# bioinformatics-ua/polus

Measured on AMD Instinct MI355X. Metric: train samples/sec BioBERT-base NER seq256, higher is better.
Workload: dtype bf16; 1 GPU; BERT-base (L=12,H=768,A=12,I=3072,V=28996) token classification C=4, seq_len=256, 64 samples/GPU, AdamW lr 5e-5 wd 0.01 warm-up 10%, dropout 0.1 (hidden + attention) (BASELINE.json configs[2] per-GPU shape), random-init weights; global_batch=64, seq_len=256, parallelism=dp1, grad_allreduce=none

## Files before the change

polus_amd/csrc/attention.hip:

```cpp
#include "common.h"

namespace {

constexpr int D = 64;
constexpr int BLK = 64;
constexpr float MASK_NEG = -10000.0f;
constexpr float LOG2E = 1.4426950408889634f, LN2 = 0.6931471805599453f;

template <typename T> struct TileCfg;
template <> struct TileCfg<bf16_t> { static constexpr int RS = 160, EPC = 8, LOG_CPR = 3, NLOAD = 2; };
template <> struct TileCfg<float> { static constexpr int RS = 288, EPC = 4, LOG_CPR = 4, NLOAD = 4; };

template <typename T, int NT = 256>
__device__ __forceinline__ void tile_load(unsigned char* tile, const T* __restrict__ base, long ld, int row0,
                                          int nrows, int col0, int tid) {
    constexpr int LOG = TileCfg<T>::LOG_CPR;
#pragma unroll
    for (int k = 0; k < TileCfg<T>::NLOAD; ++k) {
        int c = tid + NT * k;
        int r = c >> LOG, ch = c & ((1 << LOG) - 1);
        uint4 v = make_uint4(0, 0, 0, 0);
        if (row0 + r < nrows)
            v = *reinterpret_cast<const uint4*>(base + (long)(row0 + r) * ld + col0 + ch * TileCfg<T>::EPC);
        *reinterpret_cast<uint4*>(tile + r * TileCfg<T>::RS + ch * 16) = v;
    }
}

template <typename T>
__device__ __forceinline__ void frag_global(Frag<T>& f, const T* __restrict__ p, bool valid);
template <>
__device__ __forceinline__ void frag_global<bf16_t>(Frag<bf16_t>& f, const bf16_t* __restrict__ p, bool valid) {
    uint4 v = make_uint4(0, 0, 0, 0);
    if (valid) v = *reinterpret_cast<const uint4*>(p);
    f.v = __builtin_bit_cast(bf16x8, v);
}
template <>
__device__ __forceinline__ void frag_global<float>(Frag<float>& f, const float* __restrict__ p, bool valid) {
    float4 a = make_float4(0, 0, 0, 0), b = a;
    if (valid) { a = *reinterpret_cast<const float4*>(p); b = *reinterpret_cast<const float4*>(p + 4); }
    f.v[0] = a.x; f.v[1] = a.y; f.v[2] = a.z; f.v[3] = a.w;
    f.v[4] = b.x; f.v[5] = b.y; f.v[6] = b.z; f.v[7] = b.w;
}

template <typename T>
__device__ __forceinline__ void frag_row(Frag<T>& f, const unsigned char* tile, int row, int sub, int g) {
    frag_load_row(f, tile + row * TileCfg<T>::RS + (sub * 32 + 8 * g) * (int)sizeof(T));
}

__device__ __forceinline__ void frag_tr(Frag<bf16_t>& f, const unsigned char* tile, int kb, int d0, int i, int g) {
    const unsigned char* p = tile + (kb + 4 * g + (i >> 2)) * 160 + (d0 + 4 * (i & 3)) * 2;
    s16x4 lo = lds_tr16(p);
    s16x4 hi = lds_tr16(p + 16 * 160);
    typedef short s16x8 __attribute__((ext_vector_type(8)));
    s16x8 w = {lo[0], lo[1], lo[2], lo[3], hi[0], hi[1], hi[2], hi[3]};
    f.v = __builtin_bit_cast(bf16x8, w);
}
__device__ __forceinline__ void frag_tr(Frag<float>& f, const unsigned char* tile, int kb, int d0, int i, int g) {
#pragma unroll
    for (int j = 0; j < 8; ++j)
        f.v[j] = *reinterpret_cast<const float*>(tile + (kb + 16 * (j >> 2) + 4 * g + (j & 3)) * 288 + (d0 + i) * 4);
}

__device__ __forceinline__ void frag_from_acc(Frag<bf16_t>& f, const f32x4& t0, const f32x4& t1) {
    f.v[0] = (bf16_t)t0[0]; f.v[1] = (bf16_t)t0[1]; f.v[2] = (bf16_t)t0[2]; f.v[3] = (bf16_t)t0[3];
    f.v[4] = (bf16_t)t1[0]; f.v[5] = (bf16_t)t1[1]; f.v[6] = (bf16_t)t1[2]; f.v[7] = (bf16_t)t1[3];
}
__device__ __forceinline__ void frag_from_acc(Frag<float>& f, const f32x4& t0, const f32x4& t1) {
    f.v[0] = t0[0]; f.v[1] = t0[1]; f.v[2] = t0[2]; f.v[3] = t0[3];
    f.v[4] = t1[0]; f.v[5] = t1[1]; f.v[6] = t1[2]; f.v[7] = t1[3];
}

__device__ __forceinline__ float col_max(float v) { v = fmaxf(v, __shfl_xor(v, 16, 64)); return fmaxf(v, __shfl_xor(v, 32, 64)); }
__device__ __forceinline__ float col_sum(float v) { v += __shfl_xor(v, 16, 64); return v + __shfl_xor(v, 32, 64); }

template <typename T>
__device__ __forceinline__ void store_acc_T(T* __restrict__ out, long ld, int row, int col0, const f32x4 (&o)[4],
                                            float mul, int g, bool valid) {
    if (!valid) return;
#pragma unroll
    for (int dt = 0; dt < 4; ++dt) {
        float v[4] = {o[dt][0] * mul, o[dt][1] * mul, o[dt][2] * mul, o[dt][3] * mul};
        store4<T>(out + (long)row * ld + col0 + dt * 16 + 4 * g, v);
    }
}

struct AttnArgs {
    const void* qkv; const int32_t* mask; void* ctx; float* lse;
    const void* dctx; const float* delta; void* dqkv;
    int B, S, A, H;
    float scale;
    unsigned drop_thresh, drop_seed;
    float drop_inv;
    const PolusDyn* dyn;
    int debug;
};

__device__ __forceinline__ float key_bias(const int32_t* mask, int b, int S, int key) {
    if (key >= S) return -INFINITY;
    if (!mask) return 0.0f;
    return (1.0f - (float)mask[(long)b * S + key]) * MASK_NEG;
}

template <typename T, int NW>
__global__ __launch_bounds__(64 * NW) void attn_fwd_kernel(AttnArgs p) {
    if (p.drop_thresh) p.drop_seed = polus_eff_seed(p.drop_seed, p.dyn);
    constexpr int QB = 16 * NW, NT = 64 * NW;
    extern __shared__ __attribute__((aligned(16))) unsigned char smem[];
    unsigned char* Kc = smem;
    unsigned char* Vc = smem + QB * TileCfg<T>::RS;
    float* kbc = reinterpret_cast<float*>(smem + 2 * QB * TileCfg<T>::RS);
    const int tid = threadIdx.x, lane = tid & 63, wid = tid >> 6, i = lane & 15, g = lane >> 4;
    const int q0 = blockIdx.x * QB, h = blockIdx.y, b = blockIdx.z;
    const int S = p.S, H = p.H;
    const long ld = 3L * H;
    const T* qkv = static_cast<const T*>(p.qkv) + (long)b * S * ld;
    const int q = q0 + wid * 16 + i;
    const bool qvalid = q < S;

    Frag<T> qf[2];
#pragma unroll
    for (int sub = 0; sub < 2; ++sub)
        frag_global<T>(qf[sub], qkv + (long)q * ld + h * D + sub * 32 + 8 * g, qvalid);

    const float scale2 = p.scale * LOG2E;
    float m = -1e30f, l = 0.f;
    f32x4 o[4];
#pragma unroll
    for (int dt = 0; dt < 4; ++dt) o[dt] = (f32x4){0.f, 0.f, 0.f, 0.f};

    for (int kc0 = 0; kc0 < S; kc0 += QB) {
        __syncthreads();
        tile_load<T, NT>(Kc, qkv, ld, kc0, S, H + h * D, tid);
        tile_load<T, NT>(Vc, qkv, ld, kc0, S, 2 * H + h * D, tid);
        if (tid < QB) kbc[tid] = key_bias(p.mask, b, S, kc0 + tid) * LOG2E;
        __syncthreads();
      for (int kb0 = kc0; kb0 < kc0 + QB && kb0 < S; kb0 += BLK) {
        const unsigned char* Kt = Kc + (kb0 - kc0) * TileCfg<T>::RS;
        const unsigned char* Vt = Vc + (kb0 - kc0) * TileCfg<T>::RS;
        const float* kbias = kbc + (kb0 - kc0);

        f32x4 s[4];
#pragma unroll
        for (int kt = 0; kt < 4; ++kt) {
            s[kt] = (f32x4){0.f, 0.f, 0.f, 0.f};
#pragma unroll
            for (int sub = 0; sub < 2; ++sub) {
                Frag<T> a;
                frag_row<T>(a, Kt, kt * 16 + i, sub, g);
                mma16(s[kt], a, qf[sub]);
            }
        }
        float mx = -INFINITY;
#pragma unroll
        for (int kt = 0; kt < 4; ++kt)
#pragma unroll
            for (int r = 0; r < 4; ++r) {
                s[kt][r] = fmaf(s[kt][r], scale2, kbias[kt * 16 + 4 * g + r]);
                mx = fmaxf(mx, s[kt][r]);
            }
        mx = col_max(mx);
        const float m_new = fmaxf(m, mx);
        const float alpha = __builtin_amdgcn_exp2f(m - m_new);
        float rs = 0.f;
#pragma unroll
        for (int kt = 0; kt < 4; ++kt)
#pragma unroll
            for (int r = 0; r < 4; ++r) { s[kt][r] = __builtin_amdgcn_exp2f(s[kt][r] - m_new); rs += s[kt][r]; }
        rs = col_sum(rs);
        l = l * alpha + rs;
        m = m_new;
#pragma unroll
        for (int dt = 0; dt < 4; ++dt)
#pragma unroll
            for (int r = 0; r < 4; ++r) o[dt][r] *= alpha;
        if (p.drop_thresh) {
            const unsigned rowb = (((unsigned)b * p.A + h) * S + (unsigned)q) * S + kb0 + 4 * g;
#pragma unroll
            for (int kt = 0; kt < 4; ++kt) {
                float t4[4] = {s[kt][0], s[kt][1], s[kt][2], s[kt][3]};
                polus_dropout_run<4>(t4, p.drop_seed, rowb + kt * 16, p.drop_thresh, p.drop_inv, (S & 3) == 0);
                s[kt] = (f32x4){t4[0], t4[1], t4[2], t4[3]};
            }
        }
// ... 19 lines not shown
typedef const __attribute__((address_space(1))) void* gptr_t;
__device__ __forceinline__ void dma16(const void* g, unsigned char* lds) {
    __builtin_amdgcn_global_load_lds((gptr_t)g, (lds_void_t*)lds, 16, 0, 0);
}
__device__ __forceinline__ void dma4(const void* g, unsigned char* lds) {
    __builtin_amdgcn_global_load_lds((gptr_t)g, (lds_void_t*)lds, 4, 0, 0);
}
template <int N> __device__ __forceinline__ void wait_vm() { asm volatile("s_waitcnt vmcnt(%0)" :: "n"(N) : "memory"); }
__device__ __forceinline__ void wait_lgkm() { asm volatile("s_waitcnt lgkmcnt(0)" ::: "memory"); }
template <int PPW> __device__ __forceinline__ void wait_blocks_left(int left) {
    if (left >= 3) wait_vm<3 * PPW>(); else if (left == 2) wait_vm<2 * PPW>(); else if (left == 1) wait_vm<PPW>(); else wait_vm<0>();
}
__device__ __forceinline__ float xor16(float v) {
    return __builtin_bit_cast(float, __builtin_amdgcn_ds_swizzle(__builtin_bit_cast(int, v), 0x401F));
}
__device__ __forceinline__ float col_max2(float v) {
    v = fmaxf(v, xor16(v));
    return fmaxf(v, __shfl_xor(v, 32, 64));
}
__device__ __forceinline__ float col_sum2(float v) {
    v += xor16(v);
    return v + __shfl_xor(v, 32, 64);
}

constexpr int FWD_RING = 4, FWD_STAGE = 2 * BLK * 128;
constexpr int FWD_MAX_S = 1024;

template <int NW>
__global__ __launch_bounds__(64 * NW, NW == 8 ? 4 : 2) void attn_fwd_dma_kernel(AttnArgs p) {
    typedef bf16_t T;
    constexpr int QB = 16 * NW, NT = 64 * NW, PPW = 16 / NW;
    if (p.drop_thresh) p.drop_seed = polus_eff_seed(p.drop_seed, p.dyn);
    extern __shared__ __attribute__((aligned(16))) unsigned char smem[];
    unsigned char* ring = smem;
    float* kbc = reinterpret_cast<float*>(smem + FWD_RING * FWD_STAGE);
    const int tid = threadIdx.x, lane = tid & 63, i = lane & 15, g = lane >> 4;
    const int wid = __builtin_amdgcn_readfirstlane(tid >> 6);
    const int q0 = blockIdx.x * QB, h = blockIdx.y, b = blockIdx.z;
    const int S = p.S, H = p.H;
    const long ld = 3L * H;
    const T* qkv = static_cast<const T*>(p.qkv) + (long)b * S * ld;
    const int q = q0 + wid * 16 + i;
    const int r8 = lane >> 3, src_chunk = ((lane & 7) ^ r8) * 8;

    auto issue_block = [&](int j) {
        unsigned char* st = ring + (j & 3) * FWD_STAGE;
#pragma unroll
        for (int e = 0; e < PPW; ++e) {
            const int piece = wid + e * NW;
            const int row = min(j * BLK + (piece & 7) * 8 + r8, S - 1);
            dma16(qkv + (long)row * ld + (piece < 8 ? H : 2 * H) + h * D + src_chunk, st + piece * 1024);
        }
    };
    const int nblk = (S + BLK - 1) / BLK;
    if (p.mask)
        for (int k0 = wid * 64; k0 < S; k0 += 64 * NW)
            dma4(p.mask + (long)b * S + min(k0 + lane, S - 1), reinterpret_cast<unsigned char*>(kbc) + k0 * 4);
    {
        unsigned char* qs = ring + 3 * FWD_STAGE;
#pragma unroll
        for (int e = 0; e < 2; ++e) {
            const int piece = wid + e * NW;
            dma16(qkv + (long)min(q0 + piece * 8 + r8, S - 1) * ld + h * D + src_chunk, qs + piece * 1024);
        }
    }
#pragma unroll
    for (int j = 0; j < 3; ++j) if (j < nblk) issue_block(j);
    wait_blocks_left<PPW>(min(nblk, 3));
    __builtin_amdgcn_s_barrier();
    Frag<T> qf[2];
    {
        const int row = wid * 16 + i;
#pragma unroll
        for (int sub = 0; sub < 2; ++sub)
            qf[sub].v = *reinterpret_cast<const bf16x8*>(ring + 3 * FWD_STAGE + row * 128 + (((sub * 4 + g) ^ (row & 7)) * 16));
    }
    for (int t = tid; t < nblk * BLK; t += NT) {
        float bias = 0.0f;
        if (p.mask) bias = (1.0f - (float)reinterpret_cast<const int*>(kbc)[t]) * MASK_NEG;
        kbc[t] = t < S ? bias * LOG2E : -INFINITY;
    }
    wait_lgkm();
    __builtin_amdgcn_s_barrier();
    if (nblk > 3) issue_block(3);
    int issued = min(nblk, 4);

    const float scale2 = p.scale * LOG2E;
    float m = -1e30f, l = 0.f;
    f32x4 o[4];
#pragma unroll
    for (int dt = 0; dt < 4; ++dt) o[dt] = (f32x4){0.f, 0.f, 0.f, 0.f};
    const int kx = i & 7;
    const int k_off0 = i * 128 + ((g ^ kx) * 16), k_off1 = i * 128 + (((4 + g) ^ kx) * 16);
    const int vrow = 4 * g + (i >> 2), vx = vrow & 7;
    const int v_base = vrow * 128 + (i & 1) * 8, v_c = (i & 3) >> 1;

    for (int j0 = 0; j0 < nblk; j0 += 2) {
        const bool two = j0 + 1 < nblk;
        f32x4 s[2][4];
#pragma unroll
        for (int jj = 0; jj < 2; ++jj) {
            if (jj == 0 || two) {
                wait_blocks_left<PPW>(issued - 1 - (j0 + jj));
                __builtin_amdgcn_s_barrier();
                const unsigned char* Kt = ring + ((j0 + jj) & 3) * FWD_STAGE;
#pragma unroll
                for (int kt = 0; kt < 4; ++kt) {
                    s[jj][kt] = (f32x4){0.f, 0.f, 0.f, 0.f};
                    Frag<T> a0, a1;
                    a0.v = *reinterpret_cast<const bf16x8*>(Kt + kt * 2048 + k_off0);
                    a1.v = *reinterpret_cast<const bf16x8*>(Kt + kt * 2048 + k_off1);
                    mma16(s[jj][kt], a0, qf[0]);
                    mma16(s[jj][kt], a1, qf[1]);
                }
            } else {
#pragma unroll
                for (int kt = 0; kt < 4; ++kt) s[jj][kt] = (f32x4){-INFINITY, -INFINITY, -INFINITY, -INFINITY};
            }
        }
        float mx = -INFINITY;
#pragma unroll
        for (int jj = 0; jj < 2; ++jj)
            if (jj == 0 || two) {
#pragma unroll
                for (int kt = 0; kt < 4; ++kt) {
                    const f32x4 kb = *reinterpret_cast<const f32x4*>(kbc + (j0 + jj) * BLK + kt * 16 + 4 * g);
#pragma unroll
                    for (int r = 0; r < 4; ++r) s[jj][kt][r] = fmaf(s[jj][kt][r], scale2, kb[r]);
                    mx = fmaxf(mx, fmaxf(fmaxf(s[jj][kt][0], s[jj][kt][1]), fmaxf(s[jj][kt][2], s[jj][kt][3])));
                }
            }
        mx = col_max2(mx);
        const float m_new = fmaxf(m, mx);
        const float alpha = __builtin_amdgcn_exp2f(m - m_new);
        m = m_new;
        float rs = 0.f;
        Frag<T> pf[2][2];
#pragma unroll
        for (int jj = 0; jj < 2; ++jj) {
#pragma unroll
            for (int kt = 0; kt < 4; ++kt)
#pragma unroll
                for (int r = 0; r < 4; ++r) { s[jj][kt][r] = __builtin_amdgcn_exp2f(s[jj][kt][r] - m_new); rs += s[jj][kt][r]; }
            if (p.drop_thresh) {
                const unsigned rowb = (((unsigned)b * p.A + h) * S + (unsigned)q) * S + (j0 + jj) * BLK + 4 * g;
#pragma unroll
                for (int kt = 0; kt < 4; ++kt) {
                    float t4[4] = {s[jj][kt][0], s[jj][kt][1], s[jj][kt][2], s[jj][kt][3]};
                    polus_dropout_run<4>(t4, p.drop_seed, rowb + kt * 16, p.drop_thresh, p.drop_inv, (S & 3) == 0);
                    s[jj][kt] = (f32x4){t4[0], t4[1], t4[2], t4[3]};
                }
            }
            frag_from_acc(pf[jj][0], s[jj][0], s[jj][1]);
            frag_from_acc(pf[jj][1], s[jj][2], s[jj][3]);
        }
        l = l * alpha + rs;
#pragma unroll
        for (int dt = 0; dt < 4; ++dt)
#pragma unroll
            for (int r = 0; r < 4; ++r) o[dt][r] *= alpha;
#pragma unroll
        for (int jj = 0; jj < 2; ++jj) {
            if (jj == 0 || two) {
                const unsigned char* Vt = ring + ((j0 + jj) & 3) * FWD_STAGE + BLK * 128 + v_base;
#pragma unroll
                for (int ks = 0; ks < 2; ++ks)
#pragma unroll
                    for (int dt = 0; dt < 4; ++dt) {
                        const unsigned char* vp = Vt + ks * 4096 + (((2 * dt + v_c) ^ vx) * 16);
                        const s16x4 lo = lds_tr16(vp), hi = lds_tr16(vp + 16 * 128);
                        typedef short s16x8 __attribute__((ext_vector_type(8)));
                        const s16x8 w = {lo[0], lo[1], lo[2], lo[3], hi[0], hi[1], hi[2], hi[3]};
                        Frag<T> va;
                        va.v = __builtin_bit_cast(bf16x8, w);
                        mma16(o[dt], va, pf[jj][ks]);
                    }
            }
        }
        if (j0 + 4 < nblk) {
            wait_lgkm();
            __builtin_amdgcn_s_barrier();
            issue_block(j0 + 4);
            ++issued;
            if (j0 + 5 < nblk) { issue_block(j0 + 5); ++issued; }
        }
    }
    l = col_sum2(l);
    const float inv_l = 1.0f / l;
    wait_lgkm();
    __builtin_amdgcn_s_barrier();
    unsigned char* ot = ring + wid * 2048;
#pragma unroll
    for (int dt = 0; dt < 4; ++dt) {
        float v[4] = {o[dt][0] * inv_l, o[dt][1] * inv_l, o[dt][2] * inv_l, o[dt][3] * inv_l};
        store4<T>(reinterpret_cast<T*>(ot + i * 128 + (((2 * dt + (g >> 1)) ^ (i & 7)) * 16) + (g & 1) * 8), v);
    }
    wait_lgkm();
    T* ctx = static_cast<T*>(p.ctx) + (long)b * S * H;
#pragma unroll
    for (int t = 0; t < 2; ++t) {
        const int row = 8 * t + r8, qq = q0 + wid * 16 + row;
        const uint4 v = *reinterpret_cast<const uint4*>(ot + row * 128 + (lane & 7) * 16);
        if (qq < S) *reinterpret_cast<uint4*>(ctx + (long)qq * H + h * D + (((lane & 7) ^ (row & 7)) * 8)) = v;
    }
    if (q < S && g == 0) p.lse[((long)b * p.A + h) * S + q] = m * LN2 + __logf(l);
}

template <typename T, int NW>
__global__ __launch_bounds__(64 * NW) void attn_bwd_dq_kernel(AttnArgs p) {
    if (p.drop_thresh) p.drop_seed = polus_eff_seed(p.drop_seed, p.dyn);
    constexpr int QB = 16 * NW, NT = 64 * NW;
    extern __shared__ __attribute__((aligned(16))) unsigned char smem[];
    unsigned char* Kc = smem;
    unsigned char* Vc = smem + QB * TileCfg<T>::RS;
    float* kbc = reinterpret_cast<float*>(smem + 2 * QB * TileCfg<T>::RS);
    const int tid = threadIdx.x, lane = tid & 63, wid = tid >> 6, i = lane & 15, g = lane >> 4;
    const int q0 = blockIdx.x * QB, h = blockIdx.y, b = blockIdx.z;
    const int S = p.S, H = p.H;
    const long ld = 3L * H;
    const T* qkv = static_cast<const T*>(p.qkv) + (long)b * S * ld;
    const T* dctx = static_cast<const T*>(p.dctx) + (long)b * S * H;
    const int q = q0 + wid * 16 + i;
    const bool qvalid = q < S;

    Frag<T> qf[2], dof[2];
#pragma unroll
    for (int sub = 0; sub < 2; ++sub) {
        frag_global<T>(qf[sub], qkv + (long)q * ld + h * D + sub * 32 + 8 * g, qvalid);
        frag_global<T>(dof[sub], dctx + (long)q * H + h * D + sub * 32 + 8 * g, qvalid);
    }
    const long stat = ((long)b * p.A + h) * S + q;
    const float lse2 = (qvalid ? p.lse[stat] : 0.f) * LOG2E;
    const float scale2 = p.scale * LOG2E;
    float dl = 0.f;
    {
        const T* ctx = static_cast<const T*>(p.ctx) + (long)b * S * H;
#pragma unroll
        for (int sub = 0; sub < 2; ++sub) {
            Frag<T> of;
            frag_global<T>(of, ctx + (long)q * H + h * D + sub * 32 + 8 * g, qvalid);
#pragma unroll
            for (int j = 0; j < 8; ++j) dl += (float)of.v[j] * (float)dof[sub].v[j];
        }
        dl = col_sum(dl);
        if (qvalid && g == 0) const_cast<float*>(p.delta)[stat] = dl;
    }

    f32x4 dq[4];
#pragma unroll
    for (int dt = 0; dt < 4; ++dt) dq[dt] = (f32x4){0.f, 0.f, 0.f, 0.f};

    for (int kc0 = 0; kc0 < S; kc0 += QB) {
        __syncthreads();
        tile_load<T, NT>(Kc, qkv, ld, kc0, S, H + h * D, tid);
        tile_load<T, NT>(Vc, qkv, ld, kc0, S, 2 * H + h * D, tid);
        if (tid < QB) kbc[tid] = key_bias(p.mask, b, S, kc0 + tid) * LOG2E;
        __syncthreads();
      for (int kb0 = kc0; kb0 < kc0 + QB && kb0 < S; kb0 += BLK) {
        const unsigned char* Kt = Kc + (kb0 - kc0) * TileCfg<T>::RS;
        const unsigned char* Vt = Vc + (kb0 - kc0) * TileCfg<T>::RS;
        const float* kbias = kbc + (kb0 - kc0);
        f32x4 s[4], dp[4];
#pragma unroll
        for (int kt = 0; kt < 4; ++kt) {
            s[kt] = (f32x4){0.f, 0.f, 0.f, 0.f};
            dp[kt] = (f32x4){0.f, 0.f, 0.f, 0.f};
#pragma unroll
            for (int sub = 0; sub < 2; ++sub) {
                Frag<T> a;
                frag_row<T>(a, Kt, kt * 16 + i, sub, g);
                mma16(s[kt], a, qf[sub]);
// ... 240 lines not shown
            store4<T>(reinterpret_cast<T*>(Ds + st_off), dsv);
        }
        {
            Frag<T> dsb;
            frag_from_acc(dsb, s[0], s[1]);
#pragma unroll
            for (int dt = 0; dt < 4; ++dt) {
                Frag<T> ka;
                frag_tr(ka, Kt, 0, dt * 16, i, g);
                mma16(dq[dt], ka, dsb);
            }
        }
        __syncthreads();
#pragma unroll
        for (int e = 0; e < TPW; ++e) {
            const int t = wid * TPW + e;
            const int type = t >> 3, dt = (t >> 1) & 3, ktile = t & 1;
            const unsigned char* At = type ? Oc : Qc;
            const unsigned char* Bt = type ? Ps : Ds;
            f32x4 acc = (f32x4){0.f, 0.f, 0.f, 0.f};
#pragma unroll
            for (int qs = 0; qs < S / 32; ++qs) {
                Frag<T> a, bb;
                frag_tr(a, At, qs * 32, dt * 16, i, g);
                {
                    const unsigned char* bp = Bt + ktile * (S * 32) + (qs * 32 + 4 * g + (i >> 2)) * 32 + (((i & 3) ^ g) * 8);
                    const s16x4 lo = lds_tr16(bp), hi = lds_tr16(bp + 16 * 32);
                    typedef short s16x8 __attribute__((ext_vector_type(8)));
                    const s16x8 w = {lo[0], lo[1], lo[2], lo[3], hi[0], hi[1], hi[2], hi[3]};
                    bb.v = __builtin_bit_cast(bf16x8, w);
                }
                mma16(acc, a, bb);
            }
            float v[4] = {acc[0], acc[1], acc[2], acc[3]};
            store4<T>(dqkv + (long)(kb * KBLK + ktile * 16 + i) * ld + (type ? 2 * H : H) + h * D + dt * 16 + 4 * g, v);
        }
        __syncthreads();
    }
    store_acc_T<T>(dqkv, ld, q, h * D, dq, 1.0f, g, true);
}

typedef __attribute__((address_space(3))) unsigned char lds_u8;
typedef int v2i_t __attribute__((ext_vector_type(2)));
__device__ __forceinline__ unsigned lds_off(const unsigned char* p) { return (unsigned)(unsigned long)(const lds_u8*)p; }
template <int ROW16>
__device__ __forceinline__ void tr_pair_asm(Frag<bf16_t>& f, unsigned addr) {
    v2i_t lo, hi;
    asm volatile("ds_read_b64_tr_b16 %0, %2\n\tds_read_b64_tr_b16 %1, %2 offset:%3" : "=&v"(lo), "=&v"(hi) : "v"(addr), "n"(ROW16));
    typedef int v4i_t __attribute__((ext_vector_type(4)));
    const v4i_t w = {lo[0], lo[1], hi[0], hi[1]};
    f.v = __builtin_bit_cast(bf16x8, w);
}
__device__ __forceinline__ void ds_read128_asm(Frag<bf16_t>& f, unsigned addr) {
    typedef int v4i_t __attribute__((ext_vector_type(4)));
    v4i_t w;
    asm volatile("ds_read_b128 %0, %1" : "=&v"(w) : "v"(addr));
    f.v = __builtin_bit_cast(bf16x8, w);
}
__device__ __forceinline__ uint2 ds_read64_asm(unsigned addr) {
    v2i_t w;
    asm volatile("ds_read_b64 %0, %1" : "=&v"(w) : "v"(addr));
    return make_uint2((unsigned)w[0], (unsigned)w[1]);
}
__device__ __forceinline__ void lds_fence() {
    asm volatile("s_waitcnt lgkmcnt(0)" ::: "memory");
    __builtin_amdgcn_sched_barrier(0);
}
template <int R> __device__ __forceinline__ unsigned quad_bcast(unsigned v) {
    return (unsigned)__builtin_amdgcn_mov_dpp((int)v, R | (R << 2) | (R << 4) | (R << 6), 0xF, 0xF, true);
}


constexpr int Q64_KB = 64;
template <int NW> struct Q64Cfg {
    static constexpr int S = 16 * NW;
    static constexpr int OFF_O = S * 128, OFF_K = 2 * S * 128, OFF_V = OFF_K + Q64_KB * 128, OFF_P = OFF_V + Q64_KB * 128,
                         OFF_D = OFF_P + 4 * S * 32, OFF_B = OFF_D + 4 * S * 32, SMEM = OFF_B + S * 4;
};

template <int NW>
__global__ __launch_bounds__(64 * NW, 4) void attn_bwd_q64_kernel(AttnArgs p) {
    typedef bf16_t T;
    typedef Q64Cfg<NW> C;
    constexpr int S = C::S, NT = 64 * NW, NKB = S / Q64_KB;
    constexpr int KVP = 16 / NW;
    constexpr int COMBOS = NW >= 8 ? 1 : 8 / NW;
    constexpr int KTW = NW == 16 ? 2 : 4;
    if (p.drop_thresh) p.drop_seed = polus_eff_seed(p.drop_seed, p.dyn);
    extern __shared__ __attribute__((aligned(16))) unsigned char smem[];
    unsigned char* Qi = smem;
    unsigned char* Oi = smem + C::OFF_O;
    unsigned char* Kb = smem + C::OFF_K;
    unsigned char* Vb = smem + C::OFF_V;
    unsigned char* Ps = smem + C::OFF_P;
    unsigned char* Ds = smem + C::OFF_D;
    float* kbc = reinterpret_cast<float*>(smem + C::OFF_B);
    const int tid = threadIdx.x, lane = tid & 63, i = lane & 15, g = lane >> 4;
    const int wid = __builtin_amdgcn_readfirstlane(tid >> 6);
    const int h = blockIdx.x, b = blockIdx.y;
    const int H = p.H;
    const long ld = 3L * H;
    const T* qkv = static_cast<const T*>(p.qkv) + (long)b * S * ld;
    const T* dctx = static_cast<const T*>(p.dctx) + (long)b * S * H;
    T* dqkv = static_cast<T*>(p.dqkv) + (long)b * S * ld;
    const int q = wid * 16 + i;
    const int r8 = lane >> 3, src_chunk = ((lane & 7) ^ r8) * 8;

    auto issue_kv = [&](int kb) {
#pragma unroll
        for (int e = 0; e < KVP; ++e) {
            const int piece = wid + e * NW;
            const long row = (long)(kb * Q64_KB + (piece & 7) * 8 + r8) * ld + h * D + src_chunk;
            dma16(qkv + row + (piece < 8 ? H : 2 * H), (piece < 8 ? Kb : Vb) + (piece & 7) * 1024);
        }
    };
#pragma unroll
    for (int e = 0; e < 2; ++e) {
        const int piece = wid + e * NW;
        dma16(qkv + (long)(piece * 8 + r8) * ld + h * D + src_chunk, Qi + piece * 1024);
        dma16(dctx + (long)(piece * 8 + r8) * H + h * D + src_chunk, Oi + piece * 1024);
    }
    issue_kv(0);
    if (tid < S) kbc[tid] = key_bias(p.mask, b, S, tid) * LOG2E;
    const long stat = ((long)b * p.A + h) * S + q;
    const float lse2 = p.lse[stat] * LOG2E;
    const float scale2 = p.scale * LOG2E;
    Frag<T> of[2];
    {
        const T* ctx = static_cast<const T*>(p.ctx) + (long)b * S * H;
#pragma unroll
        for (int sub = 0; sub < 2; ++sub) frag_global<T>(of[sub], ctx + (long)q * H + h * D + sub * 32 + 8 * g, true);
    }
    wait_vm<0>();
    wait_lgkm();
    __builtin_amdgcn_s_barrier();
    const int qoff0 = q * 128 + ((g ^ (q & 7)) * 16), qoff1 = q * 128 + (((4 + g) ^ (q & 7)) * 16);
    float dl = 0.f;
    {
        Frag<T> dof[2];
        ds_read128_asm(dof[0], lds_off(Oi + qoff0));
        ds_read128_asm(dof[1], lds_off(Oi + qoff1));
        lds_fence();
#pragma unroll
        for (int sub = 0; sub < 2; ++sub)
#pragma unroll
            for (int j = 0; j < 8; ++j) dl += (float)of[sub].v[j] * (float)dof[sub].v[j];
        dl = col_sum(dl);
    }
    f32x4 dq[4];
#pragma unroll
    for (int dt = 0; dt < 4; ++dt) dq[dt] = (f32x4){0.f, 0.f, 0.f, 0.f};

    const int rr0 = i * 128 + ((g ^ (i & 7)) * 16), rr1 = i * 128 + (((4 + g) ^ (i & 7)) * 16);
    const int trow = 4 * g + (i >> 2), tx = trow & 7, thalf = (i & 1) * 8, tc = (i & 3) >> 1;
    const int st_w = q * 32 + ((g ^ ((q >> 2) & 3)) * 8);
    const int st_r = trow * 32 + (((i & 3) ^ g) * 8);

    for (int kb = 0; kb < NKB; ++kb) {
        f32x4 s[4];
        Frag<T> qf[2], dof[2];
        ds_read128_asm(qf[0], lds_off(Qi + qoff0));
        ds_read128_asm(qf[1], lds_off(Qi + qoff1));
        ds_read128_asm(dof[0], lds_off(Oi + qoff0));
        ds_read128_asm(dof[1], lds_off(Oi + qoff1));
        const unsigned rowb = (((unsigned)b * p.A + h) * S + (unsigned)q) * S + kb * Q64_KB + 4 * g;
#pragma unroll
        for (int kt = 0; kt < 4; ++kt) {
            Frag<T> ka[2], va[2];
            ds_read128_asm(ka[0], lds_off(Kb + kt * 2048 + rr0));
            ds_read128_asm(ka[1], lds_off(Kb + kt * 2048 + rr1));
            ds_read128_asm(va[0], lds_off(Vb + kt * 2048 + rr0));
            ds_read128_asm(va[1], lds_off(Vb + kt * 2048 + rr1));
            lds_fence();
            f32x4 dp = (f32x4){0.f, 0.f, 0.f, 0.f};
            s[kt] = (f32x4){0.f, 0.f, 0.f, 0.f};
            mma16(s[kt], ka[0], qf[0]);
            mma16(s[kt], ka[1], qf[1]);
            mma16(dp, va[0], dof[0]);
            mma16(dp, va[1], dof[1]);
            float pd[4], dsv[4];
            bool keep[4] = {true, true, true, true};
            if (p.drop_thresh) polus_keep4(p.drop_seed, rowb + kt * 16, p.drop_thresh, keep);
            const f32x4 kbv = *reinterpret_cast<const f32x4*>(kbc + kb * Q64_KB + kt * 16 + 4 * g);
#pragma unroll
            for (int r = 0; r < 4; ++r) {
                const float pr = __builtin_amdgcn_exp2f(fmaf(s[kt][r], scale2, kbv[r]) - lse2);
                const float pk = keep[r] ? pr * p.drop_inv : 0.f;
                const float dpe = keep[r] ? dp[r] * p.drop_inv : 0.f;
                pd[r] = pk;
                dsv[r] = pr * (dpe - dl) * p.scale;
                s[kt][r] = dsv[r];
            }
            store4<T>(reinterpret_cast<T*>(Ps + kt * (S * 32) + st_w), pd);
            store4<T>(reinterpret_cast<T*>(Ds + kt * (S * 32) + st_w), dsv);
        }
        {
            Frag<T> kT[2][4];
#pragma unroll
            for (int ks = 0; ks < 2; ++ks)
#pragma unroll
                for (int dt = 0; dt < 4; ++dt)
                    tr_pair_asm<16 * 128>(kT[ks][dt], lds_off(Kb + (ks * 32 + trow) * 128 + (((2 * dt + tc) ^ tx) * 16) + thalf));
            lds_fence();
#pragma unroll
            for (int ks = 0; ks < 2; ++ks) {
                Frag<T> dsb;
                frag_from_acc(dsb, s[2 * ks], s[2 * ks + 1]);
#pragma unroll
                for (int dt = 0; dt < 4; ++dt) mma16(dq[dt], kT[ks][dt], dsb);
            }
        }
        wait_lgkm();
        __builtin_amdgcn_s_barrier();
        if (kb + 1 < NKB) issue_kv(kb + 1);
#pragma unroll
        for (int c = 0; c < COMBOS; ++c) {
            const int combo = NW == 16 ? (wid >> 1) : wid * COMBOS + c;
            const int type = combo >> 2, dt = combo & 3, kt0 = NW == 16 ? (wid & 1) * 2 : 0;
            const unsigned char* At = type ? Oi : Qi;
            const unsigned char* Bt = type ? Ps : Ds;
            constexpr int QH = (S / 32) < 4 ? (S / 32) : 4;
            f32x4 acc[KTW];
#pragma unroll
            for (int k2 = 0; k2 < KTW; ++k2) acc[k2] = (f32x4){0.f, 0.f, 0.f, 0.f};
#pragma unroll
            for (int q0 = 0; q0 < S / 32; q0 += QH) {
                Frag<T> af[QH];
#pragma unroll
                for (int qs = 0; qs < QH; ++qs)
                    tr_pair_asm<16 * 128>(af[qs], lds_off(At + ((q0 + qs) * 32 + trow) * 128 + (((2 * dt + tc) ^ tx) * 16) + thalf));
#pragma unroll
                for (int k2 = 0; k2 < KTW; ++k2) {
                    Frag<T> bf[QH];
#pragma unroll
                    for (int qs = 0; qs < QH; ++qs)
                        tr_pair_asm<16 * 32>(bf[qs], lds_off(Bt + (kt0 + k2) * (S * 32) + (q0 + qs) * 32 * 32 + st_r));
                    lds_fence();
#pragma unroll
                    for (int qs = 0; qs < QH; ++qs) mma16(acc[k2], af[qs], bf[qs]);
                }
            }
#pragma unroll
            for (int k2 = 0; k2 < KTW; ++k2) {
                float v[4] = {acc[k2][0], acc[k2][1], acc[k2][2], acc[k2][3]};
                store4<T>(dqkv + (long)(kb * Q64_KB + (kt0 + k2) * 16 + i) * ld + (type ? 2 * H : H) + h * D + dt * 16 + 4 * g, v);
            }
        }
        if (kb + 1 < NKB) wait_vm<COMBOS * KTW>();
        wait_lgkm();
        __builtin_amdgcn_s_barrier();
    }
    store_acc_T<T>(dqkv, ld, q, h * D, dq, 1.0f, g, true);
}

constexpr int KR_KEYS = 256, KR_QS = 32, KR_RING = 4;
constexpr int KR_KV = KR_KEYS * 128;
constexpr int KR_SLICE = KR_QS * 128;
constexpr int KR_DS = 2 * KR_KEYS * 32;
constexpr int KR_OFF_RING = 2 * KR_KV, KR_OFF_DS = KR_OFF_RING + KR_RING * 2 * KR_SLICE, KR_OFF_DQ = KR_OFF_DS + 2 * KR_DS,
              KR_OFF_STAT = KR_OFF_DQ + 2 * KR_SLICE;

__global__ __launch_bounds__(512, 2) void attn_bwd_kres_kernel(AttnArgs p, float* __restrict__ dq_slabs) {
    typedef bf16_t T;
    constexpr int NT = 512;
    if (p.drop_thresh) p.drop_seed = polus_eff_seed(p.drop_seed, p.dyn);
    extern __shared__ __attribute__((aligned(16))) unsigned char smem[];
    unsigned char* Kimg = smem;
    unsigned char* Vimg = smem + KR_KV;
    unsigned char* ring = smem + KR_OFF_RING;
    unsigned char* dsb = smem + KR_OFF_DS;
    unsigned char* dqb = smem + KR_OFF_DQ;
    float* lsec = reinterpret_cast<float*>(smem + KR_OFF_STAT);
    const int S = p.S, H = p.H;
    float* deltac = lsec + S;
    const int tid = threadIdx.x, lane = tid & 63, i = lane & 15, g = lane >> 4;
    const int wid = __builtin_amdgcn_readfirstlane(tid >> 6);
    const int kb = blockIdx.x, h = blockIdx.y, b = blockIdx.z;
    const int key0 = kb * KR_KEYS;
    const long ld = 3L * H;
    const T* qkv = static_cast<const T*>(p.qkv) + (long)b * S * ld;
    const T* dctx = static_cast<const T*>(p.dctx) + (long)b * S * H;
    T* dqkv = static_cast<T*>(p.dqkv) + (long)b * S * ld;
    const int r8 = lane >> 3, src_chunk = ((lane & 7) ^ r8) * 8;
    const int nsl = S / KR_QS;

#pragma unroll
    for (int e = 0; e < 4; ++e) {
        const int piece = wid + 8 * e;
        const long row = (long)(key0 + piece * 8 + r8) * ld + h * D + src_chunk;
        dma16(qkv + row + H, Kimg + piece * 1024);
        dma16(qkv + row + 2 * H, Vimg + piece * 1024);
    }
    auto issue_slice = [&](int t) {
        const int q = t * KR_QS + (wid & 3) * 8 + r8;
        unsigned char* dst = ring + (t & 3) * 2 * KR_SLICE + wid * 1024;
        if (wid < 4) dma16(qkv + (long)q * ld + h * D + src_chunk, dst);
        else dma16(dctx + (long)q * H + h * D + src_chunk, dst);
    };
#pragma unroll
    for (int t = 0; t < 3; ++t) if (t < nsl) issue_slice(t);
    {
        const T* ctx = static_cast<const T*>(p.ctx) + (long)b * S * H;
        const long stat0 = ((long)b * p.A + h) * S;
        for (int q8 = wid * 8; q8 < S; q8 += 256) {
            bf16x8 o[4], d[4];
#pragma unroll
            for (int u = 0; u < 4; ++u) {
                const int q = q8 + 64 * u + r8;
                if (!(p.debug & 8)) {
                    o[u] = *reinterpret_cast<const bf16x8*>(ctx + (long)q * H + h * D + (lane & 7) * 8);
                    d[u] = *reinterpret_cast<const bf16x8*>(dctx + (long)q * H + h * D + (lane & 7) * 8);
                } else { o[u] = (bf16x8)(bf16_t)0.f; d[u] = o[u]; }
            }
            float l4[4];
            if ((lane & 7) == 0) {
#pragma unroll
                for (int u = 0; u < 4; ++u) l4[u] = p.lse[stat0 + q8 + 64 * u + r8];
            }
#pragma unroll
            for (int u = 0; u < 4; ++u) {
                float dl = 0.f;
#pragma unroll
                for (int j = 0; j < 8; ++j) dl += (float)o[u][j] * (float)d[u][j];
                dl += __builtin_bit_cast(float, __builtin_amdgcn_ds_swizzle(__builtin_bit_cast(int, dl), 0x041F));
                dl += __builtin_bit_cast(float, __builtin_amdgcn_ds_swizzle(__builtin_bit_cast(int, dl), 0x081F));
                dl += __builtin_bit_cast(float, __builtin_amdgcn_ds_swizzle(__builtin_bit_cast(int, dl), 0x101F));
                if ((lane & 7) == 0) { deltac[q8 + 64 * u + r8] = dl; lsec[q8 + 64 * u + r8] = l4[u] * LOG2E; }
            }
        }
    }
    float kb2[2];
#pragma unroll
    for (int kt = 0; kt < 2; ++kt) kb2[kt] = key_bias(p.mask, b, S, key0 + wid * 32 + kt * 16 + i) * LOG2E;
    wait_vm<0>();
    wait_lgkm();
// ... 126 lines not shown
            *reinterpret_cast<float4*>(dst) = make_float4(dq_prev[0], dq_prev[1], dq_prev[2], dq_prev[3]);
        }
        if (t >= 1 && !dq_slabs && !(p.debug & 16)) {
            const unsigned char* src = dqb + ((t - 1) & 1) * KR_SLICE;
            const int row = tid >> 4, c8 = tid & 15;
            const uint2 v = ds_read64_asm(lds_off(src + row * 128 + (((c8 >> 1) ^ (row & 7)) * 16) + (c8 & 1) * 8));
            lds_fence();
            *reinterpret_cast<uint2*>(dqkv + (long)(q0 - KR_QS + row) * ld + h * D + c8 * 4) = v;
        }
        if (t + 3 < nsl) issue_slice(t + 3);
        f32x4 dq = (f32x4){0.f, 0.f, 0.f, 0.f};
        if (!(p.debug & 1)) {
            Frag<T> dst[8];
            const unsigned base = lds_off(dsb + (t & 1) * KR_DS + ds_r);
#pragma unroll
            for (int ks = 0; ks < 8; ++ks) tr_pair_asm<16 * 32>(dst[ks], base + ks * 32 * 32);
            lds_fence();
#pragma unroll
            for (int ks = 0; ks < 8; ++ks) mma16(dq, ktr[ks], dst[ks]);
        }
        dq_prev = dq;
        if (!dq_slabs) {
            float v[4] = {dq[0], dq[1], dq[2], dq[3]};
            const int row = my_qt * 16 + i;
            store4<T>(reinterpret_cast<T*>(dqb + (t & 1) * KR_SLICE + row * 128 + (((2 * my_dt + (g >> 1)) ^ (row & 7)) * 16) + (g & 1) * 8), v);
        }
    }
    wait_lgkm();
    __builtin_amdgcn_s_barrier();
    if (dq_slabs) {
        float* dst = dq_slabs + ((long)kb * p.B * S + (long)b * S + (nsl - 1) * KR_QS + my_qt * 16 + i) * H + h * D + my_dt * 16 + 4 * g;
        *reinterpret_cast<float4*>(dst) = make_float4(dq_prev[0], dq_prev[1], dq_prev[2], dq_prev[3]);
    }
    if (!dq_slabs) {
        const unsigned char* src = dqb + ((nsl - 1) & 1) * KR_SLICE;
        const int row = tid >> 4, c8 = tid & 15;
        const uint2 v = *reinterpret_cast<const uint2*>(src + row * 128 + (((c8 >> 1) ^ (row & 7)) * 16) + (c8 & 1) * 8);
        *reinterpret_cast<uint2*>(dqkv + (long)((nsl - 1) * KR_QS + row) * ld + h * D + c8 * 4) = v;
    }
#pragma unroll
    for (int kt = 0; kt < 2; ++kt) {
        const long key = key0 + wid * 32 + kt * 16 + i;
#pragma unroll
        for (int dt = 0; dt < 4; ++dt) {
            float a[4] = {dk[dt][kt][0] * p.scale, dk[dt][kt][1] * p.scale, dk[dt][kt][2] * p.scale, dk[dt][kt][3] * p.scale};
            float c[4] = {dv[dt][kt][0], dv[dt][kt][1], dv[dt][kt][2], dv[dt][kt][3]};
            store4<T>(dqkv + key * ld + H + h * D + dt * 16 + 4 * g, a);
            store4<T>(dqkv + key * ld + 2 * H + h * D + dt * 16 + 4 * g, c);
        }
    }
}

__global__ __launch_bounds__(256) void attn_bwd_dq_finish_kernel(const float* __restrict__ slabs, bf16_t* __restrict__ dqkv,
                                                                  long rows, int H, int nkb) {
    const long n4 = rows * (H / 4);
    for (long e = (long)blockIdx.x * blockDim.x + threadIdx.x; e < n4; e += (long)gridDim.x * blockDim.x) {
        const long row = e / (H / 4);
        const int c = (int)(e - row * (H / 4)) * 4;
        float4 a = *reinterpret_cast<const float4*>(slabs + row * H + c);
        for (int k = 1; k < nkb; ++k) {
            const float4 v = *reinterpret_cast<const float4*>(slabs + ((long)k * rows + row) * H + c);
            a.x += v.x; a.y += v.y; a.z += v.z; a.w += v.w;
        }
        float v[4] = {a.x, a.y, a.z, a.w};
        store4<bf16_t>(dqkv + row * 3L * H + c, v);
    }
}

int check_common(const char* who, int dtype, int B, int S, int A, int hd) {
    POLUS_REQUIRE(dtype == POLUS_F32 || dtype == POLUS_BF16, "%s: bad dtype %d", who, dtype);
    POLUS_REQUIRE(hd == D, "%s: head_dim must be 64 (got %d)", who, hd);
    POLUS_REQUIRE(B > 0 && S > 0 && A > 0, "%s: bad shape B=%d S=%d A=%d", who, B, S, A);
    POLUS_REQUIRE(B <= 65535 && A <= 65535, "%s: B and n_heads must be <= 65535", who);
    return POLUS_OK;
}

}

namespace {
template <int WHICH, typename T, int NW>
int launch_wide_nw(const AttnArgs& a, hipStream_t st) {
    auto kern = WHICH == 0 ? attn_fwd_kernel<T, NW> : attn_bwd_dq_kernel<T, NW>;
    constexpr int QB = 16 * NW;
    const size_t lds = 2 * (size_t)QB * TileCfg<T>::RS + QB * 4;
    static bool attr_done = false;
    if (!attr_done && lds > 48 * 1024) {
        POLUS_HIP(hipFuncSetAttribute(reinterpret_cast<const void*>(kern), hipFuncAttributeMaxDynamicSharedMemorySize, (int)lds));
        attr_done = true;
    }
    dim3 grid((a.S + QB - 1) / QB, a.A, a.B);
    hipLaunchKernelGGL(kern, grid, dim3(64 * NW), lds, st, a);
    return POLUS_OK;
}
template <int NW>
int launch_fwd_dma(const AttnArgs& a, hipStream_t st) {
    auto kern = attn_fwd_dma_kernel<NW>;
    const size_t lds = FWD_RING * FWD_STAGE + (size_t)((a.S + 64 * NW - 1) / (64 * NW)) * 64 * NW * 4;
    static bool attr_done = false;
    if (!attr_done) {
        POLUS_HIP(hipFuncSetAttribute(reinterpret_cast<const void*>(kern), hipFuncAttributeMaxDynamicSharedMemorySize,
                                      FWD_RING * FWD_STAGE + (FWD_MAX_S + 64 * NW) * 4));
        attr_done = true;
    }
    hipLaunchKernelGGL(kern, dim3((a.S + 16 * NW - 1) / (16 * NW), a.A, a.B), dim3(64 * NW), lds, st, a);
    return POLUS_OK;
}
template <int NW>
int launch_q64(const AttnArgs& a, int n_heads, int B, hipStream_t st) {
    auto kern = attn_bwd_q64_kernel<NW>;
    static bool attr_done = false;
    if (!attr_done) {
        POLUS_HIP(hipFuncSetAttribute(reinterpret_cast<const void*>(kern), hipFuncAttributeMaxDynamicSharedMemorySize, Q64Cfg<NW>::SMEM));
        attr_done = true;
    }
    hipLaunchKernelGGL(kern, dim3(n_heads, B), dim3(64 * NW), Q64Cfg<NW>::SMEM, st, a);
    return POLUS_OK;
}
template <int NW>
int launch_fused(const AttnArgs& a, int n_heads, int B, size_t lds, hipStream_t st) {
    auto kern = attn_bwd_fused_kernel<NW>;
    static bool attr_done = false;
    if (!attr_done) {
        POLUS_HIP(hipFuncSetAttribute(reinterpret_cast<const void*>(kern), hipFuncAttributeMaxDynamicSharedMemorySize, (int)lds));
        attr_done = true;
    }
    hipLaunchKernelGGL(kern, dim3(n_heads, B), dim3(64 * NW), lds, st, a);
    return POLUS_OK;
}
template <int WHICH>
int launch_wide(int dtype, const AttnArgs& a, hipStream_t st) {
    if (dtype != POLUS_BF16) return launch_wide_nw<WHICH, float, 4>(a, st);
    if (a.S >= 96) return launch_wide_nw<WHICH, bf16_t, 8>(a, st);
    return launch_wide_nw<WHICH, bf16_t, 4>(a, st);
}
}

extern "C" int polus_attention_fwd(int dtype, const void* qkv, const int32_t* mask, void* ctx, float* lse,
                                   int B, int S, int n_heads, int head_dim, float drop_p, uint32_t seed, void* stream) {
    int rc = check_common("polus_attention_fwd", dtype, B, S, n_heads, head_dim);
    if (rc) return rc;
    POLUS_REQUIRE(qkv && ctx && lse, "polus_attention_fwd: null pointer");
    POLUS_REQUIRE(polus_aligned16(qkv) && polus_aligned16(ctx), "polus_attention_fwd: pointers must be 16-byte aligned");
    AttnArgs a = {};
    POLUS_REQUIRE(drop_p >= 0.f && drop_p < 1.f && (long)B * n_heads * S * S < (1LL << 32), "polus_attention_fwd: bad dropout arguments");
    a.qkv = qkv; a.mask = mask; a.ctx = ctx; a.lse = lse;
    a.B = B; a.S = S; a.A = n_heads; a.H = n_heads * D; a.scale = 0.125f;
    a.drop_thresh = drop_p > 0.f ? polus_drop_thresh(drop_p) : 0u; a.drop_seed = seed; a.drop_inv = 1.0f / (1.0f - drop_p); a.dyn = polus_dyn();
    hipStream_t st = static_cast<hipStream_t>(stream);
    int rc2;
    if (dtype == POLUS_BF16 && S <= FWD_MAX_S)
        rc2 = S >= 96 ? launch_fwd_dma<8>(a, st) : launch_fwd_dma<4>(a, st);
    else
        rc2 = launch_wide<0>(dtype, a, st);
    if (rc2 != POLUS_OK) return rc2;
    POLUS_CHECK_LAUNCH("polus_attention_fwd");
    return POLUS_OK;
}

extern "C" size_t polus_attention_bwd_workspace_bytes(int B, int S, int n_heads) {
    size_t n = (size_t)B * S * n_heads * sizeof(float);
    if (S > KR_KEYS && S % KR_KEYS == 0 && S <= 2048) n += (size_t)(S / KR_KEYS) * B * S * n_heads * D * sizeof(float);
    return n;
}

extern "C" int polus_attention_bwd(int dtype, const void* qkv, const int32_t* mask, const void* ctx,
                                   const void* dctx, const float* lse, void* dqkv,
                                   int B, int S, int n_heads, int head_dim, float drop_p, uint32_t seed,
                                   void* workspace, size_t workspace_bytes, void* stream) {
    int rc = check_common("polus_attention_bwd", dtype, B, S, n_heads, head_dim);
    if (rc) return rc;
    POLUS_REQUIRE(qkv && ctx && dctx && lse && dqkv, "polus_attention_bwd: null pointer");
    POLUS_REQUIRE(polus_aligned16(qkv) && polus_aligned16(ctx) && polus_aligned16(dctx) && polus_aligned16(dqkv),
                  "polus_attention_bwd: pointers must be 16-byte aligned");
    size_t need = polus_attention_bwd_workspace_bytes(B, S, n_heads);
    if (!workspace || workspace_bytes < need) { polus_set_error("polus_attention_bwd: workspace %zu < %zu", workspace_bytes, need); return POLUS_ERR_WORKSPACE; }
    AttnArgs a = {};
    a.qkv = qkv; a.mask = mask; a.ctx = const_cast<void*>(ctx); a.lse = const_cast<float*>(lse); a.dctx = dctx; a.dqkv = dqkv;
    a.delta = static_cast<const float*>(workspace);
    a.B = B; a.S = S; a.A = n_heads; a.H = n_heads * D; a.scale = 0.125f;
    POLUS_REQUIRE(drop_p >= 0.f && drop_p < 1.f && (long)B * n_heads * S * S < (1LL << 32), "polus_attention_bwd: bad dropout arguments");
    a.drop_thresh = drop_p > 0.f ? polus_drop_thresh(drop_p) : 0u; a.drop_seed = seed; a.drop_inv = 1.0f / (1.0f - drop_p); a.dyn = polus_dyn();
    a.debug = polus_cfg().attn_debug;
    hipStream_t st = static_cast<hipStream_t>(stream);
    dim3 grid((S + BLK - 1) / BLK, n_heads, B);
    const int kres = polus_cfg().attn_bwd_kres;
    if (dtype == POLUS_BF16 && polus_cfg().attn_fused && kres && S % KR_KEYS == 0 && S <= 2048 && (S > KR_KEYS || kres >= 2)) {
        const int nkb = S / KR_KEYS;
        float* slabs = nkb > 1 ? static_cast<float*>(workspace) + (size_t)B * S * n_heads : nullptr;
        const size_t lds = KR_OFF_STAT + 2 * (size_t)S * sizeof(float);
        static bool attr_done = false;
        if (!attr_done) {
            POLUS_HIP(hipFuncSetAttribute(reinterpret_cast<const void*>(attn_bwd_kres_kernel), hipFuncAttributeMaxDynamicSharedMemorySize, 160 * 1024));
            attr_done = true;
        }
        hipLaunchKernelGGL(attn_bwd_kres_kernel, dim3(nkb, n_heads, B), dim3(512), lds, st, a, slabs);
        POLUS_CHECK_LAUNCH("polus_attention_bwd(key-resident)");
        if (nkb > 1) {
            hipLaunchKernelGGL(attn_bwd_dq_finish_kernel, dim3(1024), dim3(256), 0, st, slabs, static_cast<bf16_t*>(dqkv), (long)B * S, a.H, nkb);
            POLUS_CHECK_LAUNCH("polus_attention_bwd(dQ slabs)");
        }
        return POLUS_OK;
    }
    const int fused = polus_cfg().attn_fused;
    if (dtype == POLUS_BF16 && fused && S == 256) {
        int rc2 = launch_q64<16>(a, n_heads, B, st);
        if (rc2 != POLUS_OK) return rc2;
        POLUS_CHECK_LAUNCH("polus_attention_bwd(one pass, 64-key blocks)");
        return POLUS_OK;
    }
    if (dtype == POLUS_BF16 && fused && (S == 64 || S == 128)) {
        const size_t lds = 2 * (size_t)S * TileCfg<bf16_t>::RS + 4 * (size_t)KBLK * TileCfg<bf16_t>::RS + 2 * (size_t)S * RSS + (size_t)S * 4;
        int rc2 = S == 128 ? launch_fused<8>(a, n_heads, B, lds, st) : launch_fused<4>(a, n_heads, B, lds, st);
        if (rc2 != POLUS_OK) return rc2;
        POLUS_CHECK_LAUNCH("polus_attention_bwd(fused)");
        return POLUS_OK;
    }
    if (dtype == POLUS_BF16) {
        { int rc2 = launch_wide<1>(dtype, a, st); if (rc2 != POLUS_OK) return rc2; }
        POLUS_CHECK_LAUNCH("polus_attention_bwd(dq)");
        hipLaunchKernelGGL(attn_bwd_dkv_kernel<bf16_t>, grid, dim3(256), 0, st, a);
    } else {
        { int rc2 = launch_wide<1>(dtype, a, st); if (rc2 != POLUS_OK) return rc2; }
        POLUS_CHECK_LAUNCH("polus_attention_bwd(dq)");
        hipLaunchKernelGGL(attn_bwd_dkv_kernel<float>, grid, dim3(256), 0, st, a);
    }
    POLUS_CHECK_LAUNCH("polus_attention_bwd(dkv)");
    return POLUS_OK;
}
```

Measured before the change: 5343 samples/s.

## Skip fully masked trailing key blocks in attention forward and backward

Scans the key padding mask with a wavefront ballot to find the last live key, then limits the forward and the one-pass backward attention loops to key blocks up to that point. dK/dV rows for the skipped padded keys are written as zeros explicitly. This removes matmul and softmax work on padded tail keys, which contribute only negligible probability (bias of -10000). The cost is a mask scan per block, and results differ slightly from the reference because the tiny exp(-10000) terms are dropped. Launch helpers also get compile-time LDS sizes as a side cleanup.

```diff
diff --git a/polus_amd/csrc/attention.hip b/polus_amd/csrc/attention.hip
--- a/polus_amd/csrc/attention.hip
+++ b/polus_amd/csrc/attention.hip
@@ -99,6 +99,22 @@
     if (key >= S) return -INFINITY;
     if (!mask) return 0.0f;
     return (1.0f - (float)mask[(long)b * S + key]) * MASK_NEG;
+}
+
+__device__ __forceinline__ int live_key_end(const float* kbc, int S, int lane) {
+    int kend = 0;
+    for (int k0 = 0; k0 < S; k0 += 64) {
+        const int k = k0 + lane;
+        const unsigned long long live = __ballot(k < S && kbc[k] != MASK_NEG * LOG2E);
+        if (live) kend = k0 + 64 - __clzll((long long)live);
+    }
+    return kend;
+}
+__device__ __forceinline__ int live_blocks(const int32_t* mask, const float* kbc, int S, int lane) {
+    const int nblk = (S + BLK - 1) / BLK;
+    if (!mask) return nblk;
+    const int kend = live_key_end(kbc, S, lane);
+    return __builtin_amdgcn_readfirstlane(kend > 0 ? (kend + BLK - 1) / BLK : nblk);
 }
 
 template <typename T, int NW>
@@ -284,8 +300,9 @@
     }
     wait_lgkm();
     __builtin_amdgcn_s_barrier();
-    if (nblk > 3) issue_block(3);
-    int issued = min(nblk, 4);
+    const int nb = live_blocks(p.mask, kbc, S, lane);
+    int issued = min(nblk, 3);
+    if (nb > 3) { issue_block(3); ++issued; }
 
     const float scale2 = p.scale * LOG2E;
     float m = -1e30f, l = 0.f;
@@ -297,8 +314,8 @@
     const int vrow = 4 * g + (i >> 2), vx = vrow & 7;
     const int v_base = vrow * 128 + (i & 1) * 8, v_c = (i & 3) >> 1;
 
-    for (int j0 = 0; j0 < nblk; j0 += 2) {
-        const bool two = j0 + 1 < nblk;
+    for (int j0 = 0; j0 < nb; j0 += 2) {
+        const bool two = j0 + 1 < nb;
         f32x4 s[2][4];
 #pragma unroll
         for (int jj = 0; jj < 2; ++jj) {
@@ -340,6 +357,7 @@
         Frag<T> pf[2][2];
 #pragma unroll
         for (int jj = 0; jj < 2; ++jj) {
+            if (jj == 1 && !two) break;
 #pragma unroll
             for (int kt = 0; kt < 4; ++kt)
 #pragma unroll
@@ -379,16 +397,17 @@
                     }
             }
         }
-        if (j0 + 4 < nblk) {
+        if (j0 + 4 < nb) {
             wait_lgkm();
             __builtin_amdgcn_s_barrier();
             issue_block(j0 + 4);
             ++issued;
-            if (j0 + 5 < nblk) { issue_block(j0 + 5); ++issued; }
+            if (j0 + 5 < nb) { issue_block(j0 + 5); ++issued; }
         }
     }
     l = col_sum2(l);
     const float inv_l = 1.0f / l;
+    wait_vm<0>();
     wait_lgkm();
     __builtin_amdgcn_s_barrier();
     unsigned char* ot = ring + wid * 2048;
@@ -795,7 +814,7 @@
 __global__ __launch_bounds__(64 * NW, 4) void attn_bwd_q64_kernel(AttnArgs p) {
     typedef bf16_t T;
     typedef Q64Cfg<NW> C;
-    constexpr int S = C::S, NT = 64 * NW, NKB = S / Q64_KB;
+    constexpr int S = C::S, NT = 64 * NW;
     constexpr int KVP = 16 / NW;
     constexpr int COMBOS = NW >= 8 ? 1 : 8 / NW;
     constexpr int KTW = NW == 16 ? 2 : 4;
@@ -847,6 +866,7 @@
     wait_vm<0>();
     wait_lgkm();
     __builtin_amdgcn_s_barrier();
+    const int nkb = live_blocks(p.mask, kbc, S, lane);
     const int qoff0 = q * 128 + ((g ^ (q & 7)) * 16), qoff1 = q * 128 + (((4 + g) ^ (q & 7)) * 16);
     float dl = 0.f;
     {
@@ -869,7 +889,7 @@
     const int st_w = q * 32 + ((g ^ ((q >> 2) & 3)) * 8);
     const int st_r = trow * 32 + (((i & 3) ^ g) * 8);
 
-    for (int kb = 0; kb < NKB; ++kb) {
+    for (int kb = 0; kb < nkb; ++kb) {
         f32x4 s[4];
         Frag<T> qf[2], dof[2];
         ds_read128_asm(qf[0], lds_off(Qi + qoff0));
@@ -925,7 +945,7 @@
         }
         wait_lgkm();
         __builtin_amdgcn_s_barrier();
-        if (kb + 1 < NKB) issue_kv(kb + 1);
+        if (kb + 1 < nkb) issue_kv(kb + 1);
 #pragma unroll
         for (int c = 0; c < COMBOS; ++c) {
             const int combo = NW == 16 ? (wid >> 1) : wid * COMBOS + c;
@@ -959,11 +979,15 @@
                 store4<T>(dqkv + (long)(kb * Q64_KB + (kt0 + k2) * 16 + i) * ld + (type ? 2 * H : H) + h * D + dt * 16 + 4 * g, v);
             }
         }
-        if (kb + 1 < NKB) wait_vm<COMBOS * KTW>();
+        if (kb + 1 < nkb) wait_vm<COMBOS * KTW>();
         wait_lgkm();
         __builtin_amdgcn_s_barrier();
     }
     store_acc_T<T>(dqkv, ld, q, h * D, dq, 1.0f, g, true);
+    for (int c = tid; c < (S - nkb * Q64_KB) * 16; c += NT) {
+        const int key = nkb * Q64_KB + (c >> 4), ch = c & 15;
+        *reinterpret_cast<uint4*>(dqkv + (long)key * ld + (ch < 8 ? H : 2 * H) + h * D + (ch & 7) * 8) = make_uint4(0, 0, 0, 0);
+    }
 }
 
 constexpr int KR_KEYS = 256, KR_QS = 32, KR_RING = 4;
@@ -1256,9 +1280,9 @@
 int launch_wide_nw(const AttnArgs& a, hipStream_t st) {
     auto kern = WHICH == 0 ? attn_fwd_kernel<T, NW> : attn_bwd_dq_kernel<T, NW>;
     constexpr int QB = 16 * NW;
-    const size_t lds = 2 * (size_t)QB * TileCfg<T>::RS + QB * 4;
+    constexpr size_t lds = 2 * (size_t)QB * TileCfg<T>::RS + QB * 4;
     static bool attr_done = false;
-    if (!attr_done && lds > 48 * 1024) {
+    if (!attr_done) {
         POLUS_HIP(hipFuncSetAttribute(reinterpret_cast<const void*>(kern), hipFuncAttributeMaxDynamicSharedMemorySize, (int)lds));
         attr_done = true;
     }
@@ -1291,8 +1315,10 @@
     return POLUS_OK;
 }
 template <int NW>
-int launch_fused(const AttnArgs& a, int n_heads, int B, size_t lds, hipStream_t st) {
+int launch_fused(const AttnArgs& a, int n_heads, int B, hipStream_t st) {
     auto kern = attn_bwd_fused_kernel<NW>;
+    constexpr int S = 16 * NW;
+    constexpr size_t lds = 2 * (size_t)S * TileCfg<bf16_t>::RS + 4 * (size_t)KBLK * TileCfg<bf16_t>::RS + 2 * (size_t)S * RSS + (size_t)S * 4;
     static bool attr_done = false;
     if (!attr_done) {
         POLUS_HIP(hipFuncSetAttribute(reinterpret_cast<const void*>(kern), hipFuncAttributeMaxDynamicSharedMemorySize, (int)lds));
@@ -1383,8 +1409,7 @@
         return POLUS_OK;
     }
     if (dtype == POLUS_BF16 && fused && (S == 64 || S == 128)) {
-        const size_t lds = 2 * (size_t)S * TileCfg<bf16_t>::RS + 4 * (size_t)KBLK * TileCfg<bf16_t>::RS + 2 * (size_t)S * RSS + (size_t)S * 4;
-        int rc2 = S == 128 ? launch_fused<8>(a, n_heads, B, lds, st) : launch_fused<4>(a, n_heads, B, lds, st);
+        int rc2 = S == 128 ? launch_fused<8>(a, n_heads, B, st) : launch_fused<4>(a, n_heads, B, st);
         if (rc2 != POLUS_OK) return rc2;
         POLUS_CHECK_LAUNCH("polus_attention_bwd(fused)");
         return POLUS_OK;
```

Result: faster. 5402 samples/s (median of 6 runs) (+1.1%).
